# Senryoku/zflac

Measured on AMD Instinct MI355X. Metric: Msamples/s decoded (bit-exact) + achieved HBM GB/s, 4096-blk stereo, higher is better.
Workload: dtype int32; 1 GPU; C5 shard: 1250 stereo 16-bit mid/side FLAC streams/GPU x 32 frames x 4096 samples, LPC order 8, partition order 4; streams_total=1250, parallelism=stream-shard x1

## Files before the change

zflac_amd/csrc/common.h:

```cpp
#pragma once
#include <cstdint>

#ifdef __HIPCC__
#define ZFLAC_HD __host__ __device__
#else
#define ZFLAC_HD
#endif

namespace zflac {

enum Err : int {
    E_OK = 0,
    E_INVALID_SIGNATURE = 1,
    E_INVALID_METADATA_HEADER = 2,
    E_MISSING_STREAMINFO = 3,
    E_UNIMPLEMENTED = 4,
    E_INVALID_CHECKSUM = 5,
    E_INVALID_FRAME_HEADER = 6,
    E_INCONSISTENT_PARAMETERS = 7,
    E_INVALID_CODED_NUMBER = 8,
    E_INVALID_SUBFRAME_HEADER = 9,
    E_INVALID_RESIDUAL_CODING = 10,
    E_END_OF_STREAM = 11,
    E_OUT_OF_MEMORY = 12,
// ... 40 lines not shown
constexpr uint64_t CHUNK_BYTES = (uint64_t)SCAN_THREADS * SCAN_BYTES_PER_THREAD;
constexpr int CHUNK_CAP = 64;
constexpr uint64_t INPUT_PAD = 4096;
constexpr int MAX_CH = 8;
#ifndef ZFLAC_WAVE_WALK_MAX_FRAMES
#define ZFLAC_WAVE_WALK_MAX_FRAMES 16384
#endif
constexpr uint64_t WAVE_WALK_MAX_FRAMES = ZFLAC_WAVE_WALK_MAX_FRAMES;
constexpr uint64_t DUMMY_BYTES = 64 * 64 * 32;
constexpr uint64_t PROBE_BYTES = 256;

struct ScanArgs {
    const uint8_t* in;
    const StreamDesc* streams;
    const ChunkDesc* chunks;
    uint32_t n_chunks;
    uint32_t* chunk_cnt;
    unsigned long long* chunk_units;
    uint64_t* chunk_slots;
    uint32_t* chunk_slot_units;
    uint32_t* status;
    uint32_t n_status;
    uint32_t* misc;
};

struct CompactArgs {
    const uint8_t* in;
    const StreamDesc* streams;
    const ChunkDesc* chunks;
    uint32_t n_chunks;
    const uint32_t* chunk_cnt;
    const uint64_t* chunk_slots;
    const uint32_t* chunk_slot_units;
    const uint32_t* chunk_off;
    const unsigned long long* chunk_uoff;
    uint32_t cap;
    uint64_t* c_pos;
    uint32_t* c_stream;
    uint64_t* c_out;
    uint32_t* overflow;
};

struct DecodeArgs {
    const uint8_t* in;
    uint64_t in_size;
    void* out;
// ... 125 lines not shown
```

zflac_amd/csrc/decode.inc:

```
#include "device_common.h"
#include "launch.h"

namespace zflac {

#ifndef ZFLAC_RING_Q
#define ZFLAC_RING_Q 16
#endif
constexpr int RING_Q = ZFLAC_RING_Q;
constexpr int RING_W = RING_Q * 4;
constexpr uint32_t RING_SLOT_MASK = (uint32_t)(RING_W - 1) << 8;
constexpr int RING_WAVE_WORDS = RING_W * 64;
constexpr int JUNK_WAVE_WORDS = 4 * 64;
#ifndef ZFLAC_DEC_THREADS
#define ZFLAC_DEC_THREADS 256
#endif
constexpr int DEC_THREADS = ZFLAC_DEC_THREADS;
#ifndef ZFLAC_WALK_THREADS
#define ZFLAC_WALK_THREADS 256
#endif
constexpr int WALK_THREADS = ZFLAC_WALK_THREADS;
constexpr int CHUNK = 32;
constexpr int DEC_CHUNK = 32;
constexpr int STAGE_SAMPLES = 32;
template <int KIND>
// ... 269 lines not shown
        else pd.flush(pend_two<KIND>());
    }
    rd.template topup<topup_quads<KIND>()>();
}

struct LaneCtx {
    uint32_t bs;
    int bps;
    int ubps;
    uint32_t chan_code;
    uint32_t end;
    int mode;
    int wasted;
    int cbps;
    int order;
    int shift;
    int32_t cval;
    int method;
    uint32_t psize;
    uint32_t parts_left;
    uint32_t left;
    uint32_t k;
    uint32_t kp1;
    uint32_t thr;
    uint32_t escw;
    bool esc;
    int err;
    bool dom;
    bool unsafe;
    uint32_t dcr;
};

template <int KIND>
__device__ __forceinline__ bool fits_sb(int64_t v) {
    if constexpr (Kind<KIND>::SB == 8) return v == (int64_t)(int8_t)v;
    else if constexpr (Kind<KIND>::SB == 16) return v == (int64_t)(int16_t)v;
    else return v == (int64_t)(int32_t)v;
}
template <int KIND>
__device__ __forceinline__ constexpr uint64_t safe_lpc_bound() {
    return KIND == 0 ? 0x7FFFull : (KIND == 1 ? (1ull << 30) : ~0ull);
}

__device__ __forceinline__ void set_err(LaneCtx& L, const Rdr& rd, int e) {
    if (!L.err) L.err = (rd.pos() > L.end) ? E_END_OF_STREAM : e;
    L.mode = M_NONE;
}

template <int KIND>
__device__ __forceinline__ void read_partition_header(LaneCtx& L, Rdr& rd) {
    const uint32_t k = rd.read(L.method ? 5 : 4);
    L.esc = k == (L.method ? 31u : 15u);
    L.k = L.esc ? 0u : k;
    L.kp1 = L.k + 1;
    L.thr = 1u << L.k;
    L.escw = 0;
    if (L.esc) {
        L.escw = rd.read(5);
        if (L.escw > (uint32_t)Kind<KIND>::W) set_err(L, rd, E_OUT_OF_DOMAIN);
    } else if (k >= (uint32_t)Kind<KIND>::W) {
        set_err(L, rd, E_OUT_OF_DOMAIN);
    }
    L.left = L.psize;
    L.parts_left--;
}

template <int KIND>
__device__ __forceinline__ void read_residual_header(LaneCtx& L, Rdr& rd) {
    const uint32_t method = rd.read(2);
    if (method >= 2) { set_err(L, rd, E_INVALID_RESIDUAL_CODING); return; }
    L.method = (int)method;
    const uint32_t po = rd.read(4);
    L.psize = L.bs >> po;
    if (L.psize < (uint32_t)L.order || (L.psize << po) != L.bs) { set_err(L, rd, E_OUT_OF_DOMAIN); return; }
    L.parts_left = 1u << po;
    read_partition_header<KIND>(L, rd);
    L.left = L.psize - (uint32_t)L.order;
}
// ... 4 lines not shown
    else if constexpr (Kind<KIND>::W == 32) return (int32_t)(((uint32_t)zz >> 1) ^ (0u - ((uint32_t)zz & 1)));
    else {
        const uint32_t z = (uint32_t)zz & 0xFFFFu;
        return (int16_t)((z >> 1) ^ (0u - (z & 1)));
    }
}

template <int KIND>
__device__ __forceinline__ int64_t rice_general(LaneCtx& L, Rdr& rd) {
    uint32_t q;
    if (!rd.unary(L.end, q)) { set_err(L, rd, E_END_OF_STREAM); return 0; }
    const uint32_t rem = rd.read(L.k);
    if constexpr (Kind<KIND>::W == 16) {
        if (q > 0xFFFFu) set_err(L, rd, E_OUT_OF_DOMAIN);
    }
    if constexpr (Kind<KIND>::W == 64) return zigzag<KIND>(((uint64_t)q << L.k) + rem);
    else return zigzag<KIND>((uint64_t)((q << L.k) + rem));
}

template <int KIND>
__device__ __forceinline__ int64_t residual_general(LaneCtx& L, Rdr& rd) {
    if (L.esc) return L.escw ? (int64_t)rd.read_signed(L.escw) : 0;
    const uint32_t h = rd.hi();
    if (h >= L.thr) {
        const uint32_t q = __builtin_clz(h);
        const uint32_t len = q + L.kp1;
        const uint32_t rem = __builtin_amdgcn_ubfe(h, 32 - len, L.k);
        rd.consume(len);
        return zigzag<KIND>((q << L.k) | rem);
    }
    return rice_general<KIND>(L, rd);
}

typedef short short2v __attribute__((ext_vector_type(2)));

template <int M>
__host__ __device__ constexpr int hist_len() { return M == 12 ? 16 : M; }

template <int KIND, int M, bool PAIRS = (KIND != 2)>
struct Pred;

template <int KIND, int M>
struct Pred<KIND, M, true> {
    static constexpr int H = hist_len<M>();
    uint32_t P[H];
    uint32_t CP[M / 2];
    int32_t last;
    __device__ __forceinline__ void clear() {
#pragma unroll
        for (int j = 0; j < H; j++) P[j] = 0;
#pragma unroll
        for (int m = 0; m < M / 2; m++) CP[m] = 0;
        last = 0;
    }
    template <int J>
    __device__ __forceinline__ void set_coef(int32_t c) {
        if constexpr ((J & 1) == 0) CP[J >> 1] = (CP[J >> 1] & 0xFFFFu) | ((uint32_t)c << 16);
        else CP[J >> 1] = (CP[J >> 1] & 0xFFFF0000u) | ((uint32_t)c & 0xFFFFu);
    }
    template <int U>
    __device__ __forceinline__ void push(int32_t s) {
        P[U % H] = __builtin_amdgcn_perm((uint32_t)s, (uint32_t)last, 0x05040100u);
        last = s;
    }
    template <int U>
    __device__ __forceinline__ uint32_t pair() const { return P[U % H]; }
    template <int U>
    __device__ __forceinline__ int32_t value() const {
        return (int32_t)(int16_t)(P[U % H] >> 16);
    }
    template <int U>
    __device__ __forceinline__ int64_t predict(int shift) const {
        int32_t acc;
        asm("v_dot2_i32_i16 %0, %1, %2, 0" : "=v"(acc) : "v"(P[(((U - 1 - 2 * (M / 2 - 1)) % H) + H) % H]), "v"(CP[M / 2 - 1]));
#pragma unroll
        for (int m = M / 2 - 2; m >= 0; m--) {
            const uint32_t a = P[(((U - 1 - 2 * m) % H) + H) % H];
            acc = __builtin_amdgcn_sdot2(__builtin_bit_cast(short2v, a), __builtin_bit_cast(short2v, CP[m]), acc,
                                         false);
        }
        if constexpr (Kind<KIND>::W == 16) acc = (int16_t)acc;
        return acc >> shift;
    }
    template <int U>
    __device__ __forceinline__ bool partials_fit(int order) const {
        constexpr int64_t HI = Kind<KIND>::W == 16 ? 0x7FFF : 0x7FFFFFFF;
        int64_t p = 0;
        bool ok = true;
#pragma unroll
// ... 12 lines not shown

template <int KIND, int M>
struct Pred<KIND, M, false> {
    static constexpr int H = hist_len<M>();
    int32_t R[H];
    int32_t C[M];
    __device__ __forceinline__ void clear() {
#pragma unroll
        for (int j = 0; j < H; j++) R[j] = 0;
#pragma unroll
        for (int j = 0; j < M; j++) C[j] = 0;
    }
    template <int J>
    __device__ __forceinline__ void set_coef(int32_t c) {
        C[J] = c;
    }
    template <int U>
    __device__ __forceinline__ void push(int32_t s) {
        R[U % H] = s;
    }
    template <int U>
    __device__ __forceinline__ int32_t value() const {
        return R[U % H];
    }
    template <int U>
    __device__ __forceinline__ int64_t predict(int shift) const {
#ifndef ZFLAC_K2_ACC
#define ZFLAC_K2_ACC 1
#endif
        constexpr int ACC = ZFLAC_K2_ACC < M - 1 ? ZFLAC_K2_ACC : M - 1;
        int64_t acc[ACC];
#pragma unroll
        for (int a = 0; a < ACC; a++) acc[a] = 0;
#pragma unroll
        for (int j = M - 1; j >= 1; j--) acc[j % ACC] += (int64_t)C[j] * (int64_t)R[(((U - 1 - j) % H) + H) % H];
#pragma unroll
        for (int a = 1; a < ACC; a++) acc[0] += acc[a];
        acc[0] += (int64_t)C[0] * (int64_t)R[(((U - 1) % H) + H) % H];
        return acc[0] >> shift;
    }
};

template <int KIND>
__device__ __forceinline__ int32_t add_inter(int64_t r, int64_t p) {
    if constexpr (Kind<KIND>::W == 16) return (int16_t)(r + p);
    else if constexpr (Kind<KIND>::W == 32) return (int32_t)((uint32_t)r + (uint32_t)p);
// ... 553 lines not shown
                                    __builtin_amdgcn_perm(b[1], b[0], 0x07030602u)),
                         make_uint4(0, 0, 0, 0));
                } else {
                    uint8_t* dst = reinterpret_cast<uint8_t*>(out) + fc.out_elem + i0;
                    emit(std::integral_constant<bool, u == L_ - 1>{}, do_store ? reinterpret_cast<uint4*>(dst) : dummy,
                         make_uint4(pk[0], pk[1], pk[2], pk[3]), make_uint4(0, 0, 0, 0));
                }
            }
        } else {
            int32_t o = KIND == 2 ? wrap_st<KIND>((int64_t)((uint64_t)(int64_t)s << wasted))
                                  : wrap_st<KIND>((int64_t)(int32_t)((uint32_t)s << wasted));
            if constexpr (LAY == LAY_STEREO) {
                int32_t x0, x1;
                pair_values(o, x0, x1);
                o = decorrelate<D_GEN>(L.chan_code, c1m, x0, x1);
                ovf |= fits_sb<KIND>(o) ? 0u : 1u;
            }
            if (do_store) store_elem<KIND>(out, fc.out_elem + (uint64_t)nch * i + c, (int32_t)((uint32_t)o << justify));
        }
    };
    if constexpr (WALK) {
        walk_steps<L_, NC, ESC, WARM>(rd, k, kp1, lim, L.esc, L.escw, wu);
        const bool dry = rd.dry();
        if constexpr (NC == 1) bad |= lim < L.thr || dry;
        else bad |= lim > 32u || dry;
        return;
    }
    uint32_t whi, wlo;
    rd.fetch(whi, wlo);
    static_for<L_ / NC>([&](auto sc) {
        constexpr int u0 = decltype(sc)::value * NC;
        uint32_t zz[NC];
        int32_t escv = 0;
        int32_t vv = 0;
        uint32_t n;
        const bool warm = WARM && (uint32_t)u0 < wu;
        const uint32_t h = rd.join(whi, wlo);
        if constexpr (MIXED) {
            const uint32_t lim0 = lim;
            n = rice_step<NC, WALK, ESC>(h, k, kp1, lim, zz, L.esc, L.escw, escv);
            if constexpr (WARM) n = warm ? 0u : n;
            vv = is_const ? (L.cval >> L.wasted) : ((int32_t)h >> vshift);
            n = is_verb ? (uint32_t)L.cbps : (is_const ? 0u : n);
            lim = (is_verb || is_const) ? lim0 : lim;
            vrange = vrange || (is_verb && !fits_sb<KIND>(vv));
        } else {
            n = rice_step<NC, WALK, ESC, RES>(h, k, kp1, lim, zz, L.esc, L.escw, escv);
            if constexpr (WARM) n = warm ? 0u : n;
        }
        rd.consume(n);
        if constexpr (decltype(sc)::value + 1 < L_ / NC) {
            rd.fetch(whi, wlo);
            __builtin_amdgcn_sched_barrier(0x6);
        }
        if constexpr (!WALK) {
            int64_t r0 = RES ? (int64_t)(int32_t)zz[0] : zigzag<KIND>(zz[0]);
            if constexpr (ESC) r0 = L.esc ? (int64_t)escv : r0;
            sample(std::integral_constant<int, u0>{}, r0, warm, vv);
            if constexpr (NC == 2)
                sample(std::integral_constant<int, u0 + 1>{}, RES ? (int64_t)(int32_t)zz[1] : zigzag<KIND>(zz[1]), false, 0);
        }
    });
    const bool dry = rd.dry();
    if constexpr (NC == 1) bad |= lim < L.thr || dry || (MIXED && vrange);
    else bad |= lim > 32u || dry;
    if constexpr (KIND == 2) vbad = v32;
    else vbad = vmax > (1 << (Kind<KIND>::SB - 1)) - 1 || vmin < -(1 << (Kind<KIND>::SB - 1));
}

template <int KIND, int M, int LAY, bool WALK, bool MIX = false>
__device__ __forceinline__ void run_subframe(LaneCtx& L, Rdr& rd, const FrameCtx& fc, void* out, int nch, int c,
                                    int32_t c1m, uint32_t bs_max, void* dummy_base) {
    constexpr int L_ = WALK ? CHUNK : DEC_CHUNK;
    static_assert(L_ % hist_len<M>() == 0 && L_ % 16 == 0, "a chunk holds whole history rings and output groups");
    uint4* const dummy = reinterpret_cast<uint4*>(dummy_base) + dummy_slot();
    Pend pd;
    pd.p = dummy;
    pd.v0 = pd.v1 = make_uint4(0, 0, 0, 0);
    StageOf<LAY> sg;
    sg.mask = 0;
    sg.base = 0;
    sg.q0 = (threadIdx.x >> 6) * STAGE_QUADS;
    uint64_t outv = reinterpret_cast<uintptr_t>(out);
    asm volatile("" : "+v"(outv));
    sg.out = reinterpret_cast<guint4*>(outv);
    if constexpr (!WALK && staged<KIND, LAY>()) {
#pragma unroll
// ... 30 lines not shown
#endif
        if (L.mode == M_PRED && base < L.bs && base >= (uint32_t)L.order && L.left == 0 && L.parts_left > 0)
            read_partition_header<KIND>(L, rd);
        if (L.mode != M_NONE && rd.pos() > L.end) set_err(L, rd, E_END_OF_STREAM);
        const bool active = L.mode != M_NONE && base < L.bs;
        uint32_t wu;
        bool lane_fast;
        if constexpr (MIX) {
            wu = base == 0 && L.mode == M_PRED ? (uint32_t)L.order : 0u;
            const bool pred_ok = L.mode == M_PRED && L.left + wu >= (uint32_t)L_ && !L.unsafe;
            const bool cv_ok = L.mode == M_CONST || (L.mode == M_VERB && L.cbps <= 32);
            lane_fast = active && base + L_ <= L.bs && (pred_ok || cv_ok) && (!need_pack || fc.packed);
        } else {
            wu = base == 0 ? (uint32_t)L.order : 0u;
            lane_fast = active && base + L_ <= fast_bs && L.mode == M_PRED && L.left + wu >= (uint32_t)L_;
        }
        const bool need_slow = active && !lane_fast;
        bool redo = __builtin_amdgcn_ballot_w64(need_slow) != 0;
#ifdef ZFLAC_PROBE
        bool was_pair = false;
#endif
        if (!redo) {
            const uint32_t k_nb = rd.nb;
            const Pred<KIND, M> k_pr = pr;
            if constexpr (!WALK) {
                sg.mask = (typename StageOf<LAY>::Mask)__builtin_amdgcn_ballot_w64(lane_fast && fc.write);
                sg.base = base;
            }
            bool bad = false;
            bool vbad = false;
            uint32_t ovf = 0;
            constexpr bool PAIRS = WALK || KIND == 1;
            const bool pairs = PAIRS && pair_cool == 0 && base != 0 &&
                               __builtin_amdgcn_ballot_w64(lane_fast && (L.k < (WALK ? 1u : 2u) || L.k > PAIR_KMAX ||
                                                                         L.esc)) == 0;
            const bool escs = __builtin_amdgcn_ballot_w64(lane_fast && L.esc) != 0;
            bool wide = false;
            if constexpr (KIND == 2 && LAY == LAY_STEREO)
                wide = __builtin_amdgcn_ballot_w64(lane_fast && L.bps > 30 && L.chan_code >= 8) != 0;
            auto fast = [&](auto decor, auto nc, auto esc) {
                fast_chunk<KIND, M, L_, LAY, decltype(decor)::value, WALK, decltype(nc)::value, decltype(esc)::value>(
                    L, rd, pr, base, fc, out, nch, c, c1m, lane_fast, dummy, bad, pd, sg, vbad, ovf);
            };
            using DGen = std::integral_constant<int, D_GEN>;
            using DMs = std::integral_constant<int, D_MS>;
            using One = std::integral_constant<int, 1>;
            using Two = std::integral_constant<int, PAIRS ? 2 : 1>;
// ... 58 lines not shown
                } else {
                    if (PAIRS && pairs) fast(DGen{}, Two{}, NoEsc{});
                    else fast(DGen{}, One{}, NoEsc{});
                }
            }
            redo = __builtin_amdgcn_ballot_w64(bad && lane_fast) != 0;
            if (PAIRS && pairs && redo) {
                pair_cool = BACKOFF ? 8u << (pair_fail < 4u ? pair_fail : 4u) : 8u;
                pair_fail++;
            } else if (BACKOFF && PAIRS && pairs) {
                pair_fail = 0;
            } else if (pair_cool) {
                pair_cool--;
            }
            pair_cool = __builtin_amdgcn_readfirstlane(pair_cool);
            if constexpr (BACKOFF) pair_fail = __builtin_amdgcn_readfirstlane(pair_fail);
#ifdef ZFLAC_PROBE
            was_pair = PAIRS && pairs && !escs && base != 0;
#endif
            if (redo || !lane_fast) {
                rd.nb = k_nb;
            }
            if (redo) {
                pr = k_pr;
                pd.p = dummy;
                sg.mask = 0;
            }
            if (!redo && lane_fast) {
                if (!MIX || L.mode == M_PRED) L.left -= L_ - wu;
                L.dom = L.dom || vbad;
                L.dcr |= ovf & (KIND == 1 ? 0x80008000u : 1u);
            }
        }
#ifdef ZFLAC_PROBE
        const uint64_t p2 = __builtin_amdgcn_s_memtime();
        const bool was_fast = !__builtin_amdgcn_ballot_w64(active && !lane_fast);
#endif
        if (redo) slow_chunk<KIND, M, L_, LAY, WALK>(L, rd, pr, base, fc, out, nch, c, c1m);
#ifdef ZFLAC_PROBE
        const uint64_t p3 = __builtin_amdgcn_s_memtime();
        pr_top += p1 - p0;
        pr_fast += p2 - p1;
        pr_slow += p3 - p2;
        pr_n += 1;
        pr_nfast += was_fast ? 1 : 0;
        pr_redo += (was_fast && redo) ? 1 : 0;
        pr_pair += was_pair ? 1 : 0;
// ... 127 lines not shown
            W.mode = M_NONE;
            if (s.frame_ok) {
                W.mode = M_PRED;
                rd.init(start);
                walk_subframe<KIND>(W, rd);
            }
            uint32_t wbs = W.mode != M_NONE ? W.bs : 0;
            for (int o = 32; o > 0; o >>= 1) wbs = max(wbs, (uint32_t)__shfl_xor((int)wbs, o));
            if (wbs) run_subframe<KIND, 4, LAY_MULTI, true>(W, rd, s.fc, a.out, nch, r, 0, wbs, a.dummy);
            start = s.frame_ok ? rd.pos() : 0u;
            if (fvalid) a.sub_start[(uint64_t)f * MAX_CH + r + 1] = start;
        }
    }
}

template <int KIND, int LAY, int MB, bool MIX>
__host__ __device__ constexpr int dec_min_waves() {
    if (MB == 32 || MIX || LAY == LAY_MULTI) return 1;
    if (KIND == 0 && MB > 8) return 1;
    if (KIND == 2 && LAY == LAY_STEREO && MB > 4) return 1;
    return 2;
}
template <int KIND, int LAY, int MB, bool MIX>
__global__ __launch_bounds__(DEC_THREADS, (dec_min_waves<KIND, LAY, MB, MIX>())) void k_decode(DecodeArgs a) {
#ifdef ZFLAC_DEC_PRIO
    __builtin_amdgcn_s_setprio(ZFLAC_DEC_PRIO);
#endif
    const int lane = threadIdx.x & 63;
    const int wave_in_block = threadIdx.x >> 6;
    const uint32_t wave = (blockIdx.x * DEC_THREADS + threadIdx.x) >> 6;
    const uint32_t nwaves = (gridDim.x * DEC_THREADS) >> 6;
    const int nch = LAY == LAY_STEREO ? 2 : (LAY == LAY_MONO ? 1 : a.nch);
    const int F = 64 / nch;
    const int c = lane / F;
    const int j = lane - c * F;
    const bool lane_ok = c < nch;
    const int32_t c1m = c ? -1 : 0;
    uint32_t nframes = a.n_frames ? *a.n_frames : a.n_frames_host;
    if (nframes > a.cap) nframes = a.cap;
    const uint32_t lds_lane = (uint32_t)(wave_in_block * RING_WAVE_WORDS + lane);

    constexpr bool FIRST = MB == 8 && !MIX;
    constexpr uint32_t MIX_BIT = 64;
    const bool rest = MB == 32 && MIX && a.rest;
    for (uint32_t g0 = wave * (uint32_t)F; g0 < nframes; g0 += nwaves * (uint32_t)F) {
        if constexpr (!FIRST) {
            const uint32_t gmb = a.group_mb[g0 / (uint32_t)F];
// ... 19 lines not shown
        }
        uint32_t ord = 0, bs_act = 0;
        bool cv = false;
        if (L.mode != M_NONE) {
            const uint32_t t = (rd.hi() >> 25) & 63;
            ord = (t >= 32) ? t - 31 : ((t >= 8 && t <= 12) ? t - 8 : 0);
            cv = t <= 1;
            bs_act = L.bs;
        }
        for (int o = 32; o > 0; o >>= 1) {
            ord = max(ord, (uint32_t)__shfl_xor((int)ord, o));
            bs_act = max(bs_act, (uint32_t)__shfl_xor((int)bs_act, o));
        }
        const bool mix = __builtin_amdgcn_ballot_w64(cv) != 0;
        const uint32_t mb = mix ? (ord <= 8 ? 8u + MIX_BIT : 32u + MIX_BIT)
                                : (ord <= 4 ? 4u : (ord <= 8 ? 8u : (ord <= 12 ? 12u : (ord <= 16 ? 16u : 32u))));
        if constexpr (FIRST) {
            if (lane == 0) {
                a.group_mb[g0 / (uint32_t)F] = mb;
                if (a.bucket_used) atomicOr(a.bucket_used, bucket_bit(mb & ~MIX_BIT, (mb & MIX_BIT) != 0));
            }
        }
        if (!rest && mb != (uint32_t)MB + (MIX ? MIX_BIT : 0u)) continue;
        run_subframe<KIND, MB, LAY, false, MIX>(L, rd, fc, a.out, nch, c, c1m, bs_act, a.dummy);

        uint32_t endbits = (rd.pos() + 7) & ~7u;
        int lerr = L.err ? L.err : (L.dom ? (int)E_OUT_OF_DOMAIN : 0);
        if (s.frame_ok && !lerr && c == nch - 1 && endbits + 16 > L.end) lerr = E_END_OF_STREAM;
        int ferr = 0;
        uint32_t dcr = 0;
        for (int cc = nch - 1; cc >= 0; cc--) {
            const int e = __shfl(lerr, cc * F + j);
            if (e) ferr = e;
            dcr |= (uint32_t)__shfl((int)L.dcr, cc * F + j);
        }
        if (LAY == LAY_STEREO && !ferr && dcr) ferr = E_OUT_OF_DOMAIN;
        const uint32_t last_end = (uint32_t)__shfl((int)endbits, (nch - 1) * F + j);
        if (fvalid && c == 0) {
            a.c_err[f] = ferr;
            a.c_info[f] = s.hdr_info;
            a.c_rate[f] = s.rate;
            a.c_end[f] = (s.pos & ~(uint64_t)15) + last_end / 8 + 2;
        }
    }
}

__host__ inline hipError_t set_lds_limit(std::atomic<uint64_t>& done, const void* fn, size_t bytes) {
    int dev = 0;
    if (const hipError_t e = hipGetDevice(&dev); e != hipSuccess) return e;
    const uint64_t bit = 1ull << (dev & 63);
    if (done.load(std::memory_order_acquire) & bit) return hipSuccess;
    const hipError_t e = hipFuncSetAttribute(fn, hipFuncAttributeMaxDynamicSharedMemorySize, (int)bytes);
    if (e == hipSuccess) done.fetch_or(bit, std::memory_order_acq_rel);
    return e;
}

template <int KIND>
hipError_t launch_walk_kind(const DecodeArgs& a, uint32_t max_frames, hipStream_t st) {
    static std::atomic<uint64_t> lds_set{0};
    if (const hipError_t e = set_lds_limit(lds_set, reinterpret_cast<const void*>(&k_walk<KIND>), WALK_LDS_BYTES);
        e != hipSuccess)
        return e;
    uint32_t waves = (max_frames + 63) / 64;
    uint32_t blocks = (waves + WALK_THREADS / 64 - 1) / (WALK_THREADS / 64);
    if (blocks > 8192) blocks = 8192;
    if (blocks == 0) blocks = 1;
    hipLaunchKernelGGL((k_walk<KIND>), dim3(blocks), dim3(WALK_THREADS), WALK_LDS_BYTES, st, a);
    return hipGetLastError();
// ... 78 lines not shown
```

zflac_amd/csrc/decode_k1_stereo.hip:

```cpp
#include "decode.inc"

namespace zflac {
hipError_t launch_decode_k1_stereo_mix(const DecodeArgs& a, uint32_t max_frames, hipStream_t st);
hipError_t launch_decode_k1_stereo(const DecodeArgs& a, uint32_t max_frames, hipStream_t st) {
    const hipError_t e = launch_decode_layout<1, LAY_STEREO>(a, max_frames, st);
    return e != hipSuccess ? e : launch_decode_k1_stereo_mix(a, max_frames, st);
}
hipError_t launch_walk_k1(const DecodeArgs& a, uint32_t max_frames, hipStream_t st) {
    return launch_walk_kind<1>(a, max_frames, st);
}
}
```

zflac_amd/csrc/pipeline.cpp:

```cpp
#include <cstdlib>
#include <cstring>
#include <functional>
#include <new>
#include <thread>
#include <unordered_map>

#include "batch.h"
#include "launch.h"

namespace zflac {
namespace {

Uploader& uploader(int device) {
    static std::mutex mu;
    static std::unordered_map<int, Uploader*> per_device;
    std::lock_guard<std::mutex> lock(mu);
    Uploader*& u = per_device[device];
    if (!u) u = new Uploader();
    return *u;
}

void fill_window(uint8_t* dst, uint64_t a, uint64_t b, const std::vector<uint64_t>& in_off,
                 const std::vector<const uint8_t*>& srcs, const std::vector<uint64_t>& lens) {
    size_t m = std::upper_bound(in_off.begin(), in_off.end(), a) - in_off.begin();
// ... 207 lines not shown
    if (C.any_unknown) {
        C.units.alloc(C.members.size());
        C.h_units = reinterpret_cast<uint64_t*>(C.pin.p + units_at);
    }
    C.cap = (uint32_t)std::min<uint64_t>(est_frames + C.chunks.size() * 2 + 1024, 0x7FFFFFFFull);
    C.est_frames = est_frames;
    C.grid_frames = (uint32_t)std::min<uint64_t>(grid_frames + grid_frames / 64 + 64, C.cap);
}

void alloc_candidates(Class& C) {
    C.c_pos.alloc(C.cap);
    C.c_out.alloc(C.cap);
    C.c_end.alloc(C.cap);
    C.c_stream.alloc(C.cap);
    C.c_info.alloc(C.cap);
    C.c_rate.alloc(C.cap);
    C.c_err.alloc(C.cap);
    C.sub.alloc((size_t)C.cap * MAX_CH);
    C.group_mb.alloc((size_t)C.cap / 4 + 2);
}

}

ScanArgs scan_args(Class& C) {
    ScanArgs a;
    std::memset(&a, 0, sizeof(a));
    a.in = C.in.p;
    a.streams = C.d_desc.p;
    a.chunks = C.d_chunks.p;
    a.n_chunks = (uint32_t)C.chunks.size();
    a.chunk_cnt = C.chunk_cnt.p;
    a.chunk_units = C.chunk_units.p;
    a.chunk_slots = C.chunk_slots.p;
    a.chunk_slot_units = C.chunk_slot_units.p;
    a.status = C.status;
    a.n_status = (uint32_t)C.members.size();
    a.misc = C.misc.p;
    return a;
}

CompactArgs compact_args(Class& C) {
    CompactArgs a;
    std::memset(&a, 0, sizeof(a));
    a.in = C.in.p;
    a.streams = C.d_desc.p;
    a.chunks = C.d_chunks.p;
    a.n_chunks = (uint32_t)C.chunks.size();
    a.chunk_cnt = C.chunk_cnt.p;
    a.chunk_slots = C.chunk_slots.p;
    a.chunk_slot_units = C.chunk_slot_units.p;
    a.chunk_off = C.chunk_off.p;
    a.chunk_uoff = C.chunk_uoff.p;
    a.cap = C.cap;
    a.c_pos = C.c_pos.p;
    a.c_stream = C.c_stream.p;
    a.c_out = C.c_out.p;
    a.overflow = C.misc.p + 1;
    return a;
}

// ... 373 lines not shown
```

zflac_amd/csrc/scan.hip:

```cpp
#include "device_common.h"
#include "launch.h"

#ifndef ZFLAC_SCAN_AUX
#define ZFLAC_SCAN_AUX 0
#endif

namespace zflac {

__device__ inline uint32_t ff_mask(uint32_t d) { return ((d & 0x7F7F7F7Fu) + 0x01010101u) & d & 0x80808080u; }

template <typename Fn>
__device__ inline void scan_window_v(const uint4 v, const uint8_t* in, uint64_t ws, uint64_t lo, uint64_t hi, Fn&& fn) {
    const uint32_t d[4] = {v.x, v.y, v.z, v.w};
#pragma unroll
    for (int k = 0; k < 4; k++) {
        uint32_t m = ff_mask(d[k]);
        while (m) {
            const int bit = __ffs(m) - 1;
            m &= m - 1;
            const int b = 4 * k + (bit >> 3);
            uint32_t nxt;
            if (b < 15) nxt = (d[(b + 1) >> 2] >> (8 * ((b + 1) & 3))) & 0xFF;
            else nxt = in[ws + 16];
            const uint64_t p = ws + b;
// ... 11 lines not shown
    const uint32_t y = (nxt & 0xFEFEFEFEu) ^ 0xF8F8F8F8u;
    const uint32_t zero = ~(((y & 0x7F7F7F7Fu) + 0x7F7F7F7Fu) | y | 0x7F7F7F7Fu);
    return ff_mask(d) & zero;
}

__device__ __forceinline__ uint32_t sync_any(uint32_t d, uint32_t dn) {
    const uint32_t nxt = __builtin_amdgcn_alignbyte(dn, d, 1);
    const uint32_t t = ~d | ((nxt & 0xFEFEFEFEu) ^ 0xF8F8F8F8u);
    return (t - 0x01010101u) & ~t & 0x80808080u;
}

__device__ __forceinline__ uint32_t lane_above(uint32_t v) {
    return (uint32_t)__builtin_amdgcn_update_dpp(0, (int)v, 0x130, 0xf, 0xf, true);
}

struct ScanLds {
    uint32_t cnt;
    unsigned long long units;
    uint64_t pos[CHUNK_CAP];
    uint32_t u[CHUNK_CAP];
};


__device__ __forceinline__ void scan_chunk(const ScanArgs& a, uint32_t chunk, ScanLds& L) {
    const ChunkDesc ch = a.chunks[chunk];
    const uint64_t abase = ch.begin & ~(uint64_t)15;
    constexpr int R = SCAN_BYTES_PER_THREAD / 16;
    const __amdgpu_buffer_rsrc_t rs = __builtin_amdgcn_make_buffer_rsrc(
        const_cast<uint8_t*>(a.in) + abase, (short)0, (int)(ch.end - abase), 0x00020000);
    uint4 v[R];
#pragma unroll
    for (int r = 0; r < R; r++)
        v[r] = __builtin_bit_cast(uint4, __builtin_amdgcn_raw_buffer_load_b128(rs, threadIdx.x * 16u,
                                                                                 r * SCAN_THREADS * 16, ZFLAC_SCAN_AUX));
    const StreamDesc S = a.streams[ch.stream];
    if (threadIdx.x == 0) {
        L.cnt = 0;
        L.units = 0;
    }
    __syncthreads();
    const uint64_t lane_ws = abase + (uint64_t)threadIdx.x * 16;
#pragma unroll
    for (int r = 0; r < R; r++) {
        const uint64_t ws = lane_ws + (uint64_t)r * SCAN_THREADS * 16;
        const uint32_t n0 = lane_above(v[r].x);
        const bool nx_mem = (threadIdx.x & 63u) == 63u || ws + 16 >= ch.end;
        const bool maybe = ((sync_any(v[r].x, v[r].y) | sync_any(v[r].y, v[r].z) | sync_any(v[r].z, v[r].w) |
                             sync_any(v[r].w, n0)) != 0 ||
                            (nx_mem && (v[r].w >> 24) == 0xFFu)) &&
                           ws < ch.end;
        if (__builtin_amdgcn_ballot_w64(maybe) == 0) continue;
#if defined(ZFLAC_SCAN_ABL) && ZFLAC_SCAN_ABL == 2
        atomicAdd(&L.cnt, 1u);
        continue;
#endif
        const uint4 vn = make_uint4(n0, lane_above(v[r].y), lane_above(v[r].z), lane_above(v[r].w));
        if (ws >= ch.end) continue;
        const uint32_t c0 = sync_mask(v[r].x, v[r].y), c1 = sync_mask(v[r].y, v[r].z),
                       c2 = sync_mask(v[r].z, v[r].w);
        uint32_t c3 = sync_mask(v[r].w, n0);
        if (nx_mem && (v[r].w >> 24) == 0xFFu)
            c3 = (c3 & 0x00808080u) | ((a.in[ws + 16] & 0xFEu) == 0xF8u ? 0x80000000u : 0u);
        if ((c0 | c1 | c2 | c3) == 0 || ws >= ch.end) continue;
#if defined(ZFLAC_SCAN_ABL) && ZFLAC_SCAN_ABL == 1
        atomicAdd(&L.cnt, (uint32_t)__builtin_popcount(c0 | c1 | c2 | c3));
        continue;
#endif
        uint32_t cand = (c0 * 0x00204081u) >> 28 & 15u;
        cand |= ((c1 * 0x00204081u) >> 28 & 15u) << 4;
        cand |= ((c2 * 0x00204081u) >> 28 & 15u) << 8;
        cand |= ((c3 * 0x00204081u) >> 28 & 15u) << 12;
        const uint4 nx = nx_mem ? *reinterpret_cast<const uint4*>(a.in + ws + 16) : vn;
        while (cand) {
            const uint32_t b = (uint32_t)__ffs(cand) - 1u;
            cand &= cand - 1u;
            const uint64_t p = ws + b;
            if (p < ch.begin || p >= ch.end) continue;
            const bool s8 = (b & 8u) != 0, s4 = (b & 4u) != 0;
            const uint32_t x0 = s8 ? v[r].z : v[r].x, x1 = s8 ? v[r].w : v[r].y, x2 = s8 ? nx.x : v[r].z,
                           x3 = s8 ? nx.y : v[r].w, x4 = s8 ? nx.z : nx.x, x5 = s8 ? nx.w : nx.y;
            const uint32_t y0 = s4 ? x1 : x0, y1 = s4 ? x2 : x1, y2 = s4 ? x3 : x2, y3 = s4 ? x4 : x3,
                           y4 = s4 ? x5 : x4;
            const uint32_t sb = b & 3u;
            const uint32_t h0 = __builtin_amdgcn_alignbyte(y1, y0, sb), h1 = __builtin_amdgcn_alignbyte(y2, y1, sb),
                           h2 = __builtin_amdgcn_alignbyte(y3, y2, sb), h3 = __builtin_amdgcn_alignbyte(y4, y3, sb);
            const FrameHdr h = parse_frame_header_t<2>(
                [h0, h1, h2, h3](uint32_t i) -> uint32_t {
                    const uint32_t sel = (i & 7u) | 0x0C0C0C00u;
                    return (i & 8u) ? __builtin_amdgcn_perm(h3, h2, sel) : __builtin_amdgcn_perm(h1, h0, sel);
                },
                S.in_end - p, S.si_rate, nullptr);
            if (!candidate_ok(h, S)) continue;
            const uint32_t slot = atomicAdd(&L.cnt, 1u);
            const uint32_t units = h.bs * S.nch;
            atomicAdd(&L.units, (unsigned long long)units);
            if (slot < CHUNK_CAP) {
                L.pos[slot] = p;
                L.u[slot] = units;
            }
        }
    }
    __syncthreads();
    if (threadIdx.x == 0) {
        const uint32_t n = L.cnt;
        const uint32_t m = n < CHUNK_CAP ? n : CHUNK_CAP;
        for (uint32_t i = 1; i < m; i++) {
            uint64_t p = L.pos[i];
            uint32_t u = L.u[i];
            int j = (int)i - 1;
            while (j >= 0 && L.pos[j] > p) {
                L.pos[j + 1] = L.pos[j];
                L.u[j + 1] = L.u[j];
                j--;
            }
            L.pos[j + 1] = p;
            L.u[j + 1] = u;
        }
    }
    __syncthreads();
}

__device__ __forceinline__ void zero_run_words(const ScanArgs& a, uint32_t chunk) {
    for (uint32_t i = chunk * SCAN_THREADS + threadIdx.x; i < a.n_status; i += a.n_chunks * SCAN_THREADS)
        a.status[i] = 0;
    if (chunk == 0 && threadIdx.x < 4) a.misc[threadIdx.x] = 0;
}

__global__ __launch_bounds__(SCAN_THREADS) void k_scan(ScanArgs a) {
    const uint32_t chunk = blockIdx.x;
    if (chunk >= a.n_chunks) return;
    zero_run_words(a, chunk);
    __shared__ ScanLds L;
    scan_chunk(a, chunk, L);
    if (threadIdx.x == 0) {
        a.chunk_cnt[chunk] = L.cnt;
        a.chunk_units[chunk] = L.units;
    }
    const uint32_t m = L.cnt < CHUNK_CAP ? L.cnt : CHUNK_CAP;
    if (threadIdx.x < m) {
        a.chunk_slots[(uint64_t)chunk * CHUNK_CAP + threadIdx.x] = L.pos[threadIdx.x];
        a.chunk_slot_units[(uint64_t)chunk * CHUNK_CAP + threadIdx.x] = L.u[threadIdx.x];
    }
}

template <typename T>
__device__ __forceinline__ T wave_incl_sum(T v) {
    const uint32_t ln = threadIdx.x & 63u;
#pragma unroll
    for (int d = 1; d < 64; d <<= 1) {
        const T y = __shfl_up(v, d, 64);
        if (ln >= (uint32_t)d) v += y;
    }
    return v;
}

constexpr int SCANK_THREADS = 1024;
constexpr int SCANK_WAVES = SCANK_THREADS / 64;
constexpr int SCANK_T = 4;

__global__ __launch_bounds__(SCANK_THREADS) void k_scan_chunks(const uint32_t* cnt, const unsigned long long* units,
                                                               uint32_t n, uint32_t* off,
                                                               unsigned long long* uoff, uint32_t* n_frames) {
    __shared__ uint32_t s_c[SCANK_WAVES];
    __shared__ unsigned long long s_u[SCANK_WAVES];
    const uint32_t t = threadIdx.x, wv = t >> 6;
// ... 110 lines not shown
                    c_pos[idx] = p;
                    c_stream[idx] = ch.stream;
                    c_out[idx] = S.out_base + (urel + ru);
                } else if (overflow) {
                    atomicOr(overflow, 1u);
                }
                rc++;
                ru += h.bs * S.nch;
            });
        }
        __syncthreads();
        if (threadIdx.x == SCAN_THREADS - 1) {
            s_base_c += s_c[threadIdx.x];
            s_base_u += s_u[threadIdx.x];
        }
        __syncthreads();
    }
}

__global__ __launch_bounds__(SCAN_THREADS) void k_compact(CompactArgs a) {
    const uint32_t c0 = blockIdx.x * COMPACT_CHUNKS;
    const uint32_t chunk = c0 + (threadIdx.x >> 6), ln = threadIdx.x & 63u;
    if (chunk < a.n_chunks) {
        const uint32_t n = a.chunk_cnt[chunk];
        if (n <= CHUNK_CAP) {
            const uint32_t stream = a.chunks[chunk].stream;
            const StreamDesc& S = a.streams[stream];
            const unsigned long long base = S.out_base + (a.chunk_uoff[chunk] - a.chunk_uoff[S.first_chunk]);
            const uint32_t u = ln < n ? a.chunk_slot_units[(uint64_t)chunk * CHUNK_CAP + ln] : 0u;
            const uint32_t pre = wave_incl_sum(u) - u;
            if (ln < n) {
                const uint32_t idx = a.chunk_off[chunk] + ln;
                if (idx < a.cap) {
                    a.c_pos[idx] = a.chunk_slots[(uint64_t)chunk * CHUNK_CAP + ln];
                    a.c_stream[idx] = stream;
                    a.c_out[idx] = base + pre;
                } else {
                    atomicOr(a.overflow, 1u);
                }
            }
        }
    }
#pragma unroll 1
    for (uint32_t j = 0; j < (uint32_t)COMPACT_CHUNKS; j++) {
        const uint32_t cj = c0 + j;
        if (cj < a.n_chunks && a.chunk_cnt[cj] > CHUNK_CAP) {
            const StreamDesc& S = a.streams[a.chunks[cj].stream];
            compact_rescan_at(a.in, a.streams, a.chunks, cj, a.chunk_off[cj],
                              a.chunk_uoff[cj] - a.chunk_uoff[S.first_chunk], a.cap, a.c_pos, a.c_stream, a.c_out,
                              a.overflow);
        }
    }
}

__global__ void k_verify(VerifyArgs a) {
    const uint32_t t = blockIdx.x * blockDim.x + threadIdx.x;
    uint32_t nframes = *a.n_frames;
// ... 29 lines not shown
        if (last && a.units) a.units[s] = end_rel;
    }
    if (bad) atomicOr(&a.status[s], 1u);
}

__global__ __launch_bounds__(SCAN_THREADS) void k_sync_list(SyncListArgs a) {
    const uint64_t abase = a.lo & ~(uint64_t)15;
    const uint64_t nwin = (a.hi - abase + 15) / 16;
    for (uint64_t w = (uint64_t)blockIdx.x * SCAN_THREADS + threadIdx.x; w < nwin;
         w += (uint64_t)gridDim.x * SCAN_THREADS) {
        scan_window(a.in, abase + w * 16, a.lo, a.hi, [&](uint64_t p) {
            const FrameHdr h = parse_frame_header(a.in + p, a.in_end - p, a.si_rate);
            if (h.err || h.crc_eof || channels_count(h.chan_code) != a.nch || h.dcode != a.dcode ||
                h.rate != a.rate_hz)
                return;
            const uint32_t slot = atomicAdd(a.count, 1u);
            if (slot < a.cap) a.pos[slot] = p;
        });
    }
}

hipError_t launch_scan(const ScanArgs& a, hipStream_t st) {
    if (a.n_chunks == 0) return hipSuccess;
    hipLaunchKernelGGL(k_scan, dim3(a.n_chunks), dim3(SCAN_THREADS), 0, st, a);
    return hipGetLastError();
}
hipError_t launch_scan_chunks(const uint32_t* cnt, const unsigned long long* units, uint32_t n, uint32_t* off,
                              unsigned long long* uoff, uint32_t* n_frames, hipStream_t st) {
    hipLaunchKernelGGL(k_scan_chunks, dim3(1), dim3(SCANK_THREADS), 0, st, cnt, units, n, off, uoff, n_frames);
    return hipGetLastError();
}
hipError_t launch_compact(const CompactArgs& a, hipStream_t st) {
    if (a.n_chunks == 0) return hipSuccess;
    hipLaunchKernelGGL(k_compact, dim3((a.n_chunks + COMPACT_CHUNKS - 1) / COMPACT_CHUNKS), dim3(SCAN_THREADS), 0, st,
                       a);
    return hipGetLastError();
}
hipError_t launch_sync_list(const SyncListArgs& a, hipStream_t st) {
    if (a.hi <= a.lo) return hipSuccess;
    const uint64_t windows = (a.hi - (a.lo & ~(uint64_t)15) + 15) / 16;
    uint64_t blocks = (windows + SCAN_THREADS - 1) / SCAN_THREADS;
    if (blocks > 4096) blocks = 4096;
    hipLaunchKernelGGL(k_sync_list, dim3((uint32_t)blocks), dim3(SCAN_THREADS), 0, st, a);
    return hipGetLastError();
}
hipError_t launch_verify(const VerifyArgs& a, uint32_t max_items, hipStream_t st) {
    uint32_t n = max_items > a.n_streams ? max_items : a.n_streams;
// ... 8 lines not shown
```

Measured before the change: 770,800 Msamples/s.

## Cap decode VGPRs for k1 stereo and add lean low-register scan kernel

Specializes the k1 stereo MB=8 decode kernel with an explicit VGPR budget and two-wave launch bound. To fit that budget it drops the stored partition threshold (recomputed from k), snapshots only the odd predictor pairs on the redo path, and writes frame info before the subframe so fewer values stay live. It also adds an opt-in lean scan kernel that uses buffer loads and global atomics with no LDS staging. The compact kernel now sorts slots by position, because the lean scan emits them out of order. The VGPR cap risks spills, and the lean scan runs only when ZFLAC_SCAN=lean is set.

New measurement: 776,500 Msamples/s (median of 6 runs). About the same (+0.7%).

```diff
diff --git a/zflac_amd/csrc/common.h b/zflac_amd/csrc/common.h
--- a/zflac_amd/csrc/common.h
+++ b/zflac_amd/csrc/common.h
@@ -86,6 +86,7 @@
     uint32_t* status;
     uint32_t n_status;
     uint32_t* misc;
+    uint32_t lean;
 };
 
 struct CompactArgs {
diff --git a/zflac_amd/csrc/decode.inc b/zflac_amd/csrc/decode.inc
--- a/zflac_amd/csrc/decode.inc
+++ b/zflac_amd/csrc/decode.inc
@@ -315,7 +315,7 @@
     uint32_t left;
     uint32_t k;
     uint32_t kp1;
-    uint32_t thr;
+    __device__ __forceinline__ uint32_t thr() const { return 1u << k; }
     uint32_t escw;
     bool esc;
     int err;
@@ -346,7 +346,6 @@
     L.esc = k == (L.method ? 31u : 15u);
     L.k = L.esc ? 0u : k;
     L.kp1 = L.k + 1;
-    L.thr = 1u << L.k;
     L.escw = 0;
     if (L.esc) {
         L.escw = rd.read(5);
@@ -397,7 +396,7 @@
 __device__ __forceinline__ int64_t residual_general(LaneCtx& L, Rdr& rd) {
     if (L.esc) return L.escw ? (int64_t)rd.read_signed(L.escw) : 0;
     const uint32_t h = rd.hi();
-    if (h >= L.thr) {
+    if (h >= L.thr()) {
         const uint32_t q = __builtin_clz(h);
         const uint32_t len = q + L.kp1;
         const uint32_t rem = __builtin_amdgcn_ubfe(h, 32 - len, L.k);
@@ -440,6 +439,23 @@
     }
     template <int U>
     __device__ __forceinline__ uint32_t pair() const { return P[U % H]; }
+    struct Snap {
+        uint32_t odd[H / 2];
+    };
+    __device__ __forceinline__ Snap snapshot() const {
+        Snap k;
+#pragma unroll
+        for (int i = 0; i < H / 2; i++) k.odd[i] = P[2 * i + 1];
+        return k;
+    }
+    __device__ __forceinline__ void restore(const Snap& k) {
+#pragma unroll
+        for (int i = 0; i < H / 2; i++) {
+            P[2 * i + 1] = k.odd[i];
+            P[2 * i] = __builtin_amdgcn_perm(k.odd[i], k.odd[(i + H / 2 - 1) % (H / 2)], 0x05040302u);
+        }
+        last = (int32_t)(int16_t)(k.odd[H / 2 - 1] >> 16);
+    }
     template <int U>
     __device__ __forceinline__ int32_t value() const {
         return (int32_t)(int16_t)(P[U % H] >> 16);
@@ -498,6 +514,19 @@
     template <int U>
     __device__ __forceinline__ int32_t value() const {
         return R[U % H];
+    }
+    struct Snap {
+        int32_t R[H];
+    };
+    __device__ __forceinline__ Snap snapshot() const {
+        Snap k;
+#pragma unroll
+        for (int j = 0; j < H; j++) k.R[j] = R[j];
+        return k;
+    }
+    __device__ __forceinline__ void restore(const Snap& k) {
+#pragma unroll
+        for (int j = 0; j < H; j++) R[j] = k.R[j];
     }
     template <int U>
     __device__ __forceinline__ int64_t predict(int shift) const {
@@ -1097,7 +1126,7 @@
     if constexpr (WALK) {
         walk_steps<L_, NC, ESC, WARM>(rd, k, kp1, lim, L.esc, L.escw, wu);
         const bool dry = rd.dry();
-        if constexpr (NC == 1) bad |= lim < L.thr || dry;
+        if constexpr (NC == 1) bad |= lim < L.thr() || dry;
         else bad |= lim > 32u || dry;
         return;
     }
@@ -1137,7 +1166,7 @@
         }
     });
     const bool dry = rd.dry();
-    if constexpr (NC == 1) bad |= lim < L.thr || dry || (MIXED && vrange);
+    if constexpr (NC == 1) bad |= lim < L.thr() || dry || (MIXED && vrange);
     else bad |= lim > 32u || dry;
     if constexpr (KIND == 2) vbad = v32;
     else vbad = vmax > (1 << (Kind<KIND>::SB - 1)) - 1 || vmin < -(1 << (Kind<KIND>::SB - 1));
@@ -1214,7 +1243,7 @@
 #endif
         if (!redo) {
             const uint32_t k_nb = rd.nb;
-            const Pred<KIND, M> k_pr = pr;
+            const typename Pred<KIND, M>::Snap k_pr = pr.snapshot();
             if constexpr (!WALK) {
                 sg.mask = (typename StageOf<LAY>::Mask)__builtin_amdgcn_ballot_w64(lane_fast && fc.write);
                 sg.base = base;
@@ -1319,7 +1348,7 @@
                 rd.nb = k_nb;
             }
             if (redo) {
-                pr = k_pr;
+                pr.restore(k_pr);
                 pd.p = dummy;
                 sg.mask = 0;
             }
@@ -1493,7 +1522,7 @@
     return 2;
 }
 template <int KIND, int LAY, int MB, bool MIX>
-__global__ __launch_bounds__(DEC_THREADS, (dec_min_waves<KIND, LAY, MB, MIX>())) void k_decode(DecodeArgs a) {
+__device__ __forceinline__ void decode_body(const DecodeArgs& a) {
 #ifdef ZFLAC_DEC_PRIO
     __builtin_amdgcn_s_setprio(ZFLAC_DEC_PRIO);
 #endif
@@ -1559,6 +1588,10 @@
             }
         }
         if (!rest && mb != (uint32_t)MB + (MIX ? MIX_BIT : 0u)) continue;
+        if (fvalid && c == 0) {
+            a.c_info[f] = s.hdr_info;
+            a.c_rate[f] = s.rate;
+        }
         run_subframe<KIND, MB, LAY, false, MIX>(L, rd, fc, a.out, nch, c, c1m, bs_act, a.dummy);
 
         uint32_t endbits = (rd.pos() + 7) & ~7u;
@@ -1575,12 +1608,21 @@
         const uint32_t last_end = (uint32_t)__shfl((int)endbits, (nch - 1) * F + j);
         if (fvalid && c == 0) {
             a.c_err[f] = ferr;
-            a.c_info[f] = s.hdr_info;
-            a.c_rate[f] = s.rate;
-            a.c_end[f] = (s.pos & ~(uint64_t)15) + last_end / 8 + 2;
-        }
-    }
-}
+            a.c_end[f] = (a.c_pos[f] & ~(uint64_t)15) + last_end / 8 + 2;
+        }
+    }
+}
+template <int KIND, int LAY, int MB, bool MIX>
+__global__ __launch_bounds__(DEC_THREADS, (dec_min_waves<KIND, LAY, MB, MIX>())) void k_decode(DecodeArgs a) {
+    decode_body<KIND, LAY, MB, MIX>(a);
+}
+
+#define ZFLAC_DECODE_VGPR_BUDGET(KIND, LAY, MB, HALF)                                                      \
+    template <>                                                                                            \
+    __global__ __launch_bounds__(DEC_THREADS, 2) __attribute__((amdgpu_num_vgpr(HALF))) void               \
+    k_decode<KIND, LAY, MB, false>(DecodeArgs a) {                                                         \
+        decode_body<KIND, LAY, MB, false>(a);                                                              \
+    }
 
 __host__ inline hipError_t set_lds_limit(std::atomic<uint64_t>& done, const void* fn, size_t bytes) {
     int dev = 0;
diff --git a/zflac_amd/csrc/decode_k1_stereo.hip b/zflac_amd/csrc/decode_k1_stereo.hip
--- a/zflac_amd/csrc/decode_k1_stereo.hip
+++ b/zflac_amd/csrc/decode_k1_stereo.hip
@@ -1,6 +1,7 @@
 #include "decode.inc"
 
 namespace zflac {
+ZFLAC_DECODE_VGPR_BUDGET(1, LAY_STEREO, 8, 116)
 hipError_t launch_decode_k1_stereo_mix(const DecodeArgs& a, uint32_t max_frames, hipStream_t st);
 hipError_t launch_decode_k1_stereo(const DecodeArgs& a, uint32_t max_frames, hipStream_t st) {
     const hipError_t e = launch_decode_layout<1, LAY_STEREO>(a, max_frames, st);
diff --git a/zflac_amd/csrc/pipeline.cpp b/zflac_amd/csrc/pipeline.cpp
--- a/zflac_amd/csrc/pipeline.cpp
+++ b/zflac_amd/csrc/pipeline.cpp
@@ -253,6 +253,11 @@
 
 }
 
+static bool use_lean_scan() {
+    const char* e = std::getenv("ZFLAC_SCAN");
+    return e && !std::strcmp(e, "lean");
+}
+
 ScanArgs scan_args(Class& C) {
     ScanArgs a;
     std::memset(&a, 0, sizeof(a));
@@ -267,6 +272,7 @@
     a.status = C.status;
     a.n_status = (uint32_t)C.members.size();
     a.misc = C.misc.p;
+    a.lean = use_lean_scan() ? 1u : 0u;
     return a;
 }
 
diff --git a/zflac_amd/csrc/scan.hip b/zflac_amd/csrc/scan.hip
--- a/zflac_amd/csrc/scan.hip
+++ b/zflac_amd/csrc/scan.hip
@@ -57,6 +57,81 @@
 };
 
 
+template <bool REG_PARSE, typename Emit>
+__device__ __forceinline__ void scan_window_syncs(const ScanArgs& a, const ChunkDesc& ch, const StreamDesc& S,
+                                                  const uint64_t ws, const uint4 v, const uint32_t n0, const bool nx_mem,
+                                                  Emit&& emit);
+template <bool REG_PARSE, typename Emit>
+__device__ __forceinline__ void scan_window_wave(const ScanArgs& a, const ChunkDesc& ch, const StreamDesc& S,
+                                                 const uint64_t ws, const uint4 v, Emit&& emit) {
+    const uint32_t n0 = lane_above(v.x);
+    const bool nx_mem = (threadIdx.x & 63u) == 63u || ws + 16 >= ch.end;
+    const bool maybe = ((sync_any(v.x, v.y) | sync_any(v.y, v.z) | sync_any(v.z, v.w) | sync_any(v.w, n0)) != 0 ||
+                        (nx_mem && (v.w >> 24) == 0xFFu)) &&
+                       ws < ch.end;
+    if (__builtin_amdgcn_ballot_w64(maybe) == 0) return;
+    scan_window_syncs<REG_PARSE>(a, ch, S, ws, v, n0, nx_mem, emit);
+}
+template <bool REG_PARSE, typename Emit>
+__device__ __forceinline__ void scan_window_syncs(const ScanArgs& a, const ChunkDesc& ch, const StreamDesc& S,
+                                                  const uint64_t ws, const uint4 v, const uint32_t n0, const bool nx_mem,
+                                                  Emit&& emit) {
+#if defined(ZFLAC_SCAN_ABL) && ZFLAC_SCAN_ABL == 2
+    emit(ws, 0u);
+    return;
+#endif
+    const uint4 vn = make_uint4(n0, lane_above(v.y), lane_above(v.z), lane_above(v.w));
+    if (ws >= ch.end) return;
+    const uint32_t c0 = sync_mask(v.x, v.y), c1 = sync_mask(v.y, v.z), c2 = sync_mask(v.z, v.w);
+    uint32_t c3 = sync_mask(v.w, n0);
+    if (nx_mem && (v.w >> 24) == 0xFFu)
+        c3 = (c3 & 0x00808080u) | ((a.in[ws + 16] & 0xFEu) == 0xF8u ? 0x80000000u : 0u);
+    if ((c0 | c1 | c2 | c3) == 0) return;
+#if defined(ZFLAC_SCAN_ABL) && ZFLAC_SCAN_ABL == 1
+    emit(ws, 0u);
+    return;
+#endif
+    uint32_t cand = (c0 * 0x00204081u) >> 28 & 15u;
+    cand |= ((c1 * 0x00204081u) >> 28 & 15u) << 4;
+    cand |= ((c2 * 0x00204081u) >> 28 & 15u) << 8;
+    cand |= ((c3 * 0x00204081u) >> 28 & 15u) << 12;
+    if constexpr (!REG_PARSE) {
+        while (cand) {
+            const uint32_t b = (uint32_t)__ffs(cand) - 1u;
+            cand &= cand - 1u;
+            const uint64_t p = ws + b;
+            if (p < ch.begin || p >= ch.end) continue;
+            const FrameHdr h = parse_frame_header(a.in + p, S.in_end - p, S.si_rate);
+            if (!candidate_ok(h, S)) continue;
+            emit(p, h.bs * S.nch);
+        }
+        return;
+    }
+    const uint4 nx = nx_mem ? *reinterpret_cast<const uint4*>(a.in + ws + 16) : vn;
+    while (cand) {
+        const uint32_t b = (uint32_t)__ffs(cand) - 1u;
+        cand &= cand - 1u;
+        const uint64_t p = ws + b;
+        if (p < ch.begin || p >= ch.end) continue;
+        const bool s8 = (b & 8u) != 0, s4 = (b & 4u) != 0;
+        const uint32_t x0 = s8 ? v.z : v.x, x1 = s8 ? v.w : v.y, x2 = s8 ? nx.x : v.z, x3 = s8 ? nx.y : v.w,
+                       x4 = s8 ? nx.z : nx.x, x5 = s8 ? nx.w : nx.y;
+        const uint32_t y0 = s4 ? x1 : x0, y1 = s4 ? x2 : x1, y2 = s4 ? x3 : x2, y3 = s4 ? x4 : x3,
+                       y4 = s4 ? x5 : x4;
+        const uint32_t sb = b & 3u;
+        const uint32_t h0 = __builtin_amdgcn_alignbyte(y1, y0, sb), h1 = __builtin_amdgcn_alignbyte(y2, y1, sb),
+                       h2 = __builtin_amdgcn_alignbyte(y3, y2, sb), h3 = __builtin_amdgcn_alignbyte(y4, y3, sb);
+        const FrameHdr h = parse_frame_header_t<2>(
+            [h0, h1, h2, h3](uint32_t i) -> uint32_t {
+                const uint32_t sel = (i & 7u) | 0x0C0C0C00u;
+                return (i & 8u) ? __builtin_amdgcn_perm(h3, h2, sel) : __builtin_amdgcn_perm(h1, h0, sel);
+            },
+            S.in_end - p, S.si_rate, nullptr);
+        if (!candidate_ok(h, S)) continue;
+        emit(p, h.bs * S.nch);
+    }
+}
+
 __device__ __forceinline__ void scan_chunk(const ScanArgs& a, uint32_t chunk, ScanLds& L) {
     const ChunkDesc ch = a.chunks[chunk];
     const uint64_t abase = ch.begin & ~(uint64_t)15;
@@ -77,63 +152,14 @@
     const uint64_t lane_ws = abase + (uint64_t)threadIdx.x * 16;
 #pragma unroll
     for (int r = 0; r < R; r++) {
-        const uint64_t ws = lane_ws + (uint64_t)r * SCAN_THREADS * 16;
-        const uint32_t n0 = lane_above(v[r].x);
-        const bool nx_mem = (threadIdx.x & 63u) == 63u || ws + 16 >= ch.end;
-        const bool maybe = ((sync_any(v[r].x, v[r].y) | sync_any(v[r].y, v[r].z) | sync_any(v[r].z, v[r].w) |
-                             sync_any(v[r].w, n0)) != 0 ||
-                            (nx_mem && (v[r].w >> 24) == 0xFFu)) &&
-                           ws < ch.end;
-        if (__builtin_amdgcn_ballot_w64(maybe) == 0) continue;
-#if defined(ZFLAC_SCAN_ABL) && ZFLAC_SCAN_ABL == 2
-        atomicAdd(&L.cnt, 1u);
-        continue;
-#endif
-        const uint4 vn = make_uint4(n0, lane_above(v[r].y), lane_above(v[r].z), lane_above(v[r].w));
-        if (ws >= ch.end) continue;
-        const uint32_t c0 = sync_mask(v[r].x, v[r].y), c1 = sync_mask(v[r].y, v[r].z),
-                       c2 = sync_mask(v[r].z, v[r].w);
-        uint32_t c3 = sync_mask(v[r].w, n0);
-        if (nx_mem && (v[r].w >> 24) == 0xFFu)
-            c3 = (c3 & 0x00808080u) | ((a.in[ws + 16] & 0xFEu) == 0xF8u ? 0x80000000u : 0u);
-        if ((c0 | c1 | c2 | c3) == 0 || ws >= ch.end) continue;
-#if defined(ZFLAC_SCAN_ABL) && ZFLAC_SCAN_ABL == 1
-        atomicAdd(&L.cnt, (uint32_t)__builtin_popcount(c0 | c1 | c2 | c3));
-        continue;
-#endif
-        uint32_t cand = (c0 * 0x00204081u) >> 28 & 15u;
-        cand |= ((c1 * 0x00204081u) >> 28 & 15u) << 4;
-        cand |= ((c2 * 0x00204081u) >> 28 & 15u) << 8;
-        cand |= ((c3 * 0x00204081u) >> 28 & 15u) << 12;
-        const uint4 nx = nx_mem ? *reinterpret_cast<const uint4*>(a.in + ws + 16) : vn;
-        while (cand) {
-            const uint32_t b = (uint32_t)__ffs(cand) - 1u;
-            cand &= cand - 1u;
-            const uint64_t p = ws + b;
-            if (p < ch.begin || p >= ch.end) continue;
-            const bool s8 = (b & 8u) != 0, s4 = (b & 4u) != 0;
-            const uint32_t x0 = s8 ? v[r].z : v[r].x, x1 = s8 ? v[r].w : v[r].y, x2 = s8 ? nx.x : v[r].z,
-                           x3 = s8 ? nx.y : v[r].w, x4 = s8 ? nx.z : nx.x, x5 = s8 ? nx.w : nx.y;
-            const uint32_t y0 = s4 ? x1 : x0, y1 = s4 ? x2 : x1, y2 = s4 ? x3 : x2, y3 = s4 ? x4 : x3,
-                           y4 = s4 ? x5 : x4;
-            const uint32_t sb = b & 3u;
-            const uint32_t h0 = __builtin_amdgcn_alignbyte(y1, y0, sb), h1 = __builtin_amdgcn_alignbyte(y2, y1, sb),
-                           h2 = __builtin_amdgcn_alignbyte(y3, y2, sb), h3 = __builtin_amdgcn_alignbyte(y4, y3, sb);
-            const FrameHdr h = parse_frame_header_t<2>(
-                [h0, h1, h2, h3](uint32_t i) -> uint32_t {
-                    const uint32_t sel = (i & 7u) | 0x0C0C0C00u;
-                    return (i & 8u) ? __builtin_amdgcn_perm(h3, h2, sel) : __builtin_amdgcn_perm(h1, h0, sel);
-                },
-                S.in_end - p, S.si_rate, nullptr);
-            if (!candidate_ok(h, S)) continue;
+        scan_window_wave<true>(a, ch, S, lane_ws + (uint64_t)r * SCAN_THREADS * 16, v[r], [&](uint64_t p, uint32_t units) {
             const uint32_t slot = atomicAdd(&L.cnt, 1u);
-            const uint32_t units = h.bs * S.nch;
             atomicAdd(&L.units, (unsigned long long)units);
             if (slot < CHUNK_CAP) {
                 L.pos[slot] = p;
                 L.u[slot] = units;
             }
-        }
+        });
     }
     __syncthreads();
     if (threadIdx.x == 0) {
@@ -176,6 +202,53 @@
         a.chunk_slots[(uint64_t)chunk * CHUNK_CAP + threadIdx.x] = L.pos[threadIdx.x];
         a.chunk_slot_units[(uint64_t)chunk * CHUNK_CAP + threadIdx.x] = L.u[threadIdx.x];
     }
+}
+
+constexpr int LEAN_AHEAD = 2;
+constexpr int LEAN_VGPRS = 48;
+
+__global__ __launch_bounds__(SCAN_THREADS) __attribute__((amdgpu_num_vgpr(24))) void k_scan_lean(ScanArgs a) {
+    static_assert(LEAN_VGPRS == 2 * 24, "the attribute states half of LEAN_VGPRS");
+    const uint32_t chunk = blockIdx.x;
+    if (chunk >= a.n_chunks) return;
+    zero_run_words(a, chunk);
+    if (threadIdx.x == 0) {
+        const uint32_t c_old = atomicExch(&a.chunk_cnt[chunk], 0u);
+        const unsigned long long u_old = atomicExch(&a.chunk_units[chunk], 0ull);
+        asm volatile("" ::"v"(c_old), "v"(u_old));
+    }
+    const ChunkDesc ch = a.chunks[chunk];
+    const uint64_t abase = ch.begin & ~(uint64_t)15;
+    constexpr int R = SCAN_BYTES_PER_THREAD / 16;
+    const __amdgpu_buffer_rsrc_t rs = __builtin_amdgcn_make_buffer_rsrc(
+        const_cast<uint8_t*>(a.in) + abase, (short)0, (int)(ch.end - abase), 0x00020000);
+    auto row = [&](int r) {
+        return __builtin_bit_cast(uint4, __builtin_amdgcn_raw_buffer_load_b128(rs, threadIdx.x * 16u,
+                                                                                r * SCAN_THREADS * 16, ZFLAC_SCAN_AUX));
+    };
+    uint4 w[LEAN_AHEAD + 1];
+#pragma unroll
+    for (int r = 0; r < LEAN_AHEAD; r++) w[r] = row(r);
+    const StreamDesc S = a.streams[ch.stream];
+    __syncthreads();
+    const uint64_t lane_ws = abase + (uint64_t)threadIdx.x * 16;
+    unsigned long long units_lane = 0;
+#pragma unroll
+    for (int r = 0; r < R; r++) {
+        if (r + LEAN_AHEAD < R) w[(r + LEAN_AHEAD) % (LEAN_AHEAD + 1)] = row(r + LEAN_AHEAD);
+        scan_window_wave<false>(a, ch, S, lane_ws + (uint64_t)r * SCAN_THREADS * 16, w[r % (LEAN_AHEAD + 1)],
+                                [&](uint64_t p, uint32_t units) {
+                                    const uint32_t slot = atomicAdd(&a.chunk_cnt[chunk], 1u);
+                                    units_lane += units;
+                                    if (slot < CHUNK_CAP) {
+                                        a.chunk_slots[(uint64_t)chunk * CHUNK_CAP + slot] = p;
+                                        a.chunk_slot_units[(uint64_t)chunk * CHUNK_CAP + slot] = units;
+                                    }
+                                });
+    }
+    if (__builtin_amdgcn_ballot_w64(units_lane != 0) == 0) return;
+    for (int o = 32; o > 0; o >>= 1) units_lane += __shfl_xor(units_lane, o);
+    if ((threadIdx.x & 63u) == 0) atomicAdd(&a.chunk_units[chunk], units_lane);
 }
 
 template <typename T>
@@ -332,17 +405,26 @@
     const uint32_t c0 = blockIdx.x * COMPACT_CHUNKS;
     const uint32_t chunk = c0 + (threadIdx.x >> 6), ln = threadIdx.x & 63u;
     if (chunk < a.n_chunks) {
-        const uint32_t n = a.chunk_cnt[chunk];
+        const uint32_t n = __builtin_amdgcn_readfirstlane(a.chunk_cnt[chunk]);
         if (n <= CHUNK_CAP) {
             const uint32_t stream = a.chunks[chunk].stream;
             const StreamDesc& S = a.streams[stream];
             const unsigned long long base = S.out_base + (a.chunk_uoff[chunk] - a.chunk_uoff[S.first_chunk]);
             const uint32_t u = ln < n ? a.chunk_slot_units[(uint64_t)chunk * CHUNK_CAP + ln] : 0u;
-            const uint32_t pre = wave_incl_sum(u) - u;
+            const uint64_t p = ln < n ? a.chunk_slots[(uint64_t)chunk * CHUNK_CAP + ln] : ~0ull;
+            uint32_t rank = 0, pre = 0;
+            for (uint32_t j = 0; j < n; j++) {
+                const uint64_t pj = __shfl(p, (int)j);
+                const uint32_t uj = __shfl(u, (int)j);
+                if (pj < p) {
+                    rank++;
+                    pre += uj;
+                }
+            }
             if (ln < n) {
-                const uint32_t idx = a.chunk_off[chunk] + ln;
+                const uint32_t idx = a.chunk_off[chunk] + rank;
                 if (idx < a.cap) {
-                    a.c_pos[idx] = a.chunk_slots[(uint64_t)chunk * CHUNK_CAP + ln];
+                    a.c_pos[idx] = p;
                     a.c_stream[idx] = stream;
                     a.c_out[idx] = base + pre;
                 } else {
@@ -418,7 +500,8 @@
 
 hipError_t launch_scan(const ScanArgs& a, hipStream_t st) {
     if (a.n_chunks == 0) return hipSuccess;
-    hipLaunchKernelGGL(k_scan, dim3(a.n_chunks), dim3(SCAN_THREADS), 0, st, a);
+    if (a.lean) hipLaunchKernelGGL(k_scan_lean, dim3(a.n_chunks), dim3(SCAN_THREADS), 0, st, a);
+    else hipLaunchKernelGGL(k_scan, dim3(a.n_chunks), dim3(SCAN_THREADS), 0, st, a);
     return hipGetLastError();
 }
 hipError_t launch_scan_chunks(const uint32_t* cnt, const unsigned long long* units, uint32_t n, uint32_t* off,
```
